# NVlabs/WarpConvNet

Measured on AMD Instinct MI355X. Metric: M active voxels/sec fwd+bwd, SparseConv3d 64→128 k=3, 1/2/4/8 MI355X, higher is better.
Workload: dtype bf16; 1 GPU; configs[1]: one 1000000-voxel uniform (U) scene per GPU, SparseConv3d 64->128 k=3, bf16 autocast, kernel-map build + AB fwd + ABt dgrad + AtB wgrad per step; voxels_per_gpu=1000000, coord_order=generator, parallelism=dp1 (scene-sharded, grad all-reduce)

## Files before the change

### warpconvnet_amd/csrc/kmap_binned.hip

```cpp
#include "kmap_cells.h"

namespace wcn {

constexpr int kInsertSample = 8;
constexpr int kInsertThreads = 512;
constexpr int kRowBufPitch = 66;
constexpr int kRowBufInts = (kCompactPitch + 1) * kRowBufPitch;
#ifndef WCN_NB_WPE
#define WCN_NB_WPE 3
#endif
constexpr int kNbWavesPerSimd = WCN_NB_WPE;
constexpr int kNbThreads = 256;

__device__ __forceinline__ int wrap_blk(int v) {
  const int bits = kBlkCoordBits;
  v &= (1 << bits) - 1;
  return (v ^ (1 << (bits - 1))) - (1 << (bits - 1));
}

__global__ void cell_prepare_kernel(uint4* __restrict__ slots, int64_t capacity, int32_t* __restrict__ ctr,
                                    uint32_t* __restrict__ halo, CellGeom g, int32_t* __restrict__ status) {
  const int64_t i = (int64_t)blockIdx.x * blockDim.x + threadIdx.x;
  if (i < capacity) slots[i] = make_uint4(0u, 0u, 0xFFFFFFFFu, 0u);
  if (i < 64) ctr[i] = 0;
  if (i == 0) *status = 0;
  if (i < g.halo_cells) {
    const int h3[3] = {g.hx, g.hy, g.hz};
    int t = (int)i, dir = 0;
    int sx = 0, sy = 0, sz = 0;
    for (; dir < 27; ++dir) {
      if (dir == 13) continue;
      const int dd[3] = {dir / 9 - 1, (dir / 3) % 3 - 1, dir % 3 - 1};
      sx = dd[0] ? h3[0] : kBlk; sy = dd[1] ? h3[1] : kBlk; sz = dd[2] ? h3[2] : kBlk;
      const int cells = sx * sy * sz;
      if (t < cells) break;
      t -= cells;
    }
    const int ddx = dir / 9 - 1, ddy = (dir / 3) % 3 - 1, ddz = dir % 3 - 1;
    const int tz = t % sz, ty = (t / sz) % sy, tx = t / (sz * sy);
    const int lx = ddx < 0 ? kBlk - g.hx + tx : tx;
    const int ly = ddy < 0 ? kBlk - g.hy + ty : ty;
    const int lz = ddz < 0 ? kBlk - g.hz + tz : tz;
    const int X = lx + kBlk * ddx + g.hx, Y = ly + kBlk * ddy + g.hy, Z = lz + kBlk * ddz + g.hz;
    halo[i] = ((uint32_t)dir << 27) | ((uint32_t)((lx * kBlk + ly) * kBlk + lz) << 16) | (uint32_t)(X * g.px + Y * g.py + Z);
  }
}

__device__ __forceinline__ void store_cell(int32_t* cell, int row, bool strict) {
  if (strict) __hip_atomic_fetch_min(reinterpret_cast<uint32_t*>(cell), (uint32_t)row, __ATOMIC_RELAXED, __HIP_MEMORY_SCOPE_AGENT);
  else *cell = row;
}

__device__ __forceinline__ int cell_of(const int4& c) {
  return ((c.y & (kBlk - 1)) * kBlk + (c.z & (kBlk - 1))) * kBlk + (c.w & (kBlk - 1));
}

template <int PHASE>
__global__ __launch_bounds__(kInsertThreads) void cell_insert_kernel(BSlot* __restrict__ slots, uint32_t cmask,
                                                          const int4* __restrict__ coords, int64_t n, CellTable t,
                                                          int32_t* __restrict__ status, int kp, int mw,
                                                          int32_t* __restrict__ nbr, uint32_t* __restrict__ mask,
                                                          int strict) {
  const bool compact = kp < 0;
  kp &= 0x7FFFFFFF;
  const int64_t tid = (int64_t)blockIdx.x * blockDim.x + threadIdx.x;
  const int64_t i = PHASE == 0 ? tid * kInsertSample : tid;
  const int lane = threadIdx.x & 63;
  bool live = i < n;
  int4 c = make_int4(0, 0, 0, 0);
  if (live) {
    c = coords[i];
    if (!coord_in_range(c.x, c.y, c.z, c.w)) {
      live = false;
      if (PHASE == 1) {
        atomicOr(status, (int)WCN_FLAG_COORD_RANGE);
        for (int k = 0; k < kp; ++k) nbr[i * kp + k] = compact ? 0 : -1;
        for (int w = 0; w < mw; ++w) mask[i * mw + w] = 0u;
      }
    }
  }
  int found = -1;
  int id = -1;
  bool created = false;
  uint64_t key = 0;
  if (live) {
    key = pack_key(c.x, c.y >> kBlkShift, c.z >> kBlkShift, c.w >> kBlkShift);
    uint32_t s = hash_slot(key, cmask);
    int idv = -1;
    for (uint32_t a = 0; a <= cmask; ++a) {
      unsigned long long* kptr = reinterpret_cast<unsigned long long*>(&slots[s].key);
      const uint4 v = *reinterpret_cast<const uint4*>(slots + s);
      unsigned long long cur = ((unsigned long long)v.y << 32) | v.x;
      if (cur == key) { found = (int)s; idv = (int)v.z; break; }
      if (cur == 0ull) {
        if (PHASE == 1) cur = __hip_atomic_load(kptr, __ATOMIC_RELAXED, __HIP_MEMORY_SCOPE_AGENT);
        if (cur == 0ull) {
          cur = atomicCAS(kptr, 0ull, (unsigned long long)key);
          if (cur == 0ull) {
            created = true;
            found = (int)s;
            break;
          }
// ... 43 lines not shown
      slots[found].id = my_id | (PHASE == 1 ? kIdLateBit : 0);
    }
    unsigned long long todo = makers;
    while (todo != 0ull) {
      const int src = __ffsll((long long)todo) - 1;
      todo &= todo - 1ull;
      const int bid = __shfl(my_id, src);
      if (bid >= 0) {
        int4* gcells = reinterpret_cast<int4*>(t.cells + (int64_t)bid * kCells);
        gcells[lane] = make_int4(-1, -1, -1, -1);
        gcells[lane + 64] = make_int4(-1, -1, -1, -1);
      }
    }
  }
  if (PHASE == 0) return;
  if (live) mask[i * mw + (mw - 1)] = (id >= 0 || found < 0) ? kMaskUnwritten : kMaskDeferred;
  if (id >= 0) store_cell(t.cells + (int64_t)id * kCells + cell_of(c), (int)i, strict != 0);
}

__global__ __launch_bounds__(256) void cell_finish_kernel(const BSlot* __restrict__ slots, uint32_t cmask,
                                                          const int4* __restrict__ coords, int64_t n, CellTable t,
                                                          CellGeom g, int mw, const uint32_t* __restrict__ mask,
                                                          int strict) {
  const int64_t tid = (int64_t)blockIdx.x * blockDim.x + threadIdx.x;
  const int64_t nthreads = (int64_t)gridDim.x * blockDim.x;
  for (int64_t i = tid; i < n; i += nthreads) {
    if (mask[i * mw + (mw - 1)] != kMaskDeferred) continue;
    const int4 c = coords[i];
    const int s = block_find(slots, cmask, pack_key(c.x, c.y >> kBlkShift, c.z >> kBlkShift, c.w >> kBlkShift));
    const int id = s >= 0 ? slots[s].id : -1;
    if (id < 0) continue;
    store_cell(t.cells + (int64_t)(id & ~kIdLateBit) * kCells + cell_of(c), (int)i, strict != 0);
  }
  const int lane = threadIdx.x & 63;
  int nblocks = t.ctr[0];
  if (nblocks > t.max_blocks) nblocks = (int)t.max_blocks;
  for (int64_t seq = tid >> 6; seq < nblocks; seq += nthreads >> 6) {
    const int id = (int)seq;
    int nid = -1;
    if (lane < 27) {
      const int ddx = lane / 9 - 1, ddy = (lane / 3) % 3 - 1, ddz = lane % 3 - 1;
      const bool needed = (ddx == 0 || g.hx > 0) && (ddy == 0 || g.hy > 0) && (ddz == 0 || g.hz > 0);
      if (lane == 13) nid = id;
      else if (needed) {
        const uint64_t key = t.blk_key[id];
        const int b = (int)((key >> 54) & kBatchMask);
        const int bx = wrap_blk((int)((key >> 36) & kCoordMask));
        const int by = wrap_blk((int)((key >> 18) & kCoordMask));
        const int bz = wrap_blk((int)(key & kCoordMask));
        const int s = block_find(slots, cmask, pack_key(b, wrap_blk(bx + ddx), wrap_blk(by + ddy), wrap_blk(bz + ddz)));
        if (s >= 0) {
          nid = slots[s].id;
          if (nid >= 0) nid &= ~kIdLateBit;
        }
      }
    }
    if (lane < 32) t.nbtab[(int64_t)id * 32 + lane] = nid;
  }
}

#ifdef WCN_PROF
__device__ unsigned long long g_bprof[4096 * 12];
#define BSTAMP(i) do { const unsigned long long now_ = wall_clock64(); prof_acc[i] += now_ - prof_prev; prof_prev = now_; } while (0)
#else
#define BSTAMP(i)
#endif

template <int LPR, bool FAST, bool COMPACT>
__global__ __launch_bounds__(kNbThreads) __attribute__((amdgpu_waves_per_eu(kNbWavesPerSimd))) void cell_neighbors_kernel(CellTable t, const uint32_t* __restrict__ halo,
                                                                    CellGeom g, int K, int kp, int mw,
                                                                    int32_t* __restrict__ nbr,
                                                                    uint32_t* __restrict__ mask,
                                                                    int32_t* __restrict__ status) {
  extern __shared__ int s_mem[];
  const int lane = threadIdx.x & 63, wave = threadIdx.x >> 6;
  uint32_t* s_halo = reinterpret_cast<uint32_t*>(s_mem);
  const int rounds = (g.halo_cells + 63) >> 6;
  const bool halo_regs = COMPACT && rounds <= 8;
  const int halo_pad = halo_regs ? 0 : rounds * 64;
  const int per_wave = g.cells + 4 + kCells / 2 + 8 + (COMPACT ? kRowBufInts : 0);
  int* s_grid = s_mem + halo_pad + wave * per_wave;
  unsigned short* s_own = reinterpret_cast<unsigned short*>(s_grid + g.cells + 4);
  const int null_cell = g.cells;
  for (int h = threadIdx.x; h < halo_pad; h += blockDim.x) s_halo[h] = h < g.halo_cells ? halo[h] : 0xFFFFFFFFu;
  if (lane == 0) s_grid[null_cell] = -1;
  __syncthreads();

  int nblocks = t.ctr[0];
  if (nblocks > t.max_blocks) nblocks = (int)t.max_blocks;
  const int gwave = blockIdx.x * (blockDim.x / 64) + wave;
  const int nwaves = gridDim.x * (blockDim.x / 64);
  constexpr int kVoxPerIter = 64 / LPR;
  const int sub = lane % LPR, vsel = lane / LPR;
  const int num_chunks = (kp + LPR - 1) / LPR;
  uint32_t he[8];
#pragma unroll
  for (int u = 0; u < 8; ++u) {
    const int idx = u * 64 + lane;
    uint32_t e = COMPACT && idx < g.halo_cells ? halo[idx] : 0xFFFFFFFFu;
    if (e == 0xFFFFFFFFu) e = (31u << 27) | (uint32_t)(g.cells + 1);
    he[u] = e;
  }
  auto load_head = [&](int seq, int& nb, int4& v0, int4& v1) {
    nb = -1;
    v0 = make_int4(-1, -1, -1, -1);
    v1 = v0;
    if (seq < nblocks) {
      if (lane < 27) nb = t.nbtab[(int64_t)seq * 32 + lane];
      const int4* own = reinterpret_cast<const int4*>(t.cells + (int64_t)seq * kCells) + lane * 2;
      v0 = own[0];
      v1 = own[1];
    }
  };
  int seq = gwave;
  int nb_c, nb_n;
  int4 c0, c1, n0, n1;
  load_head(seq, nb_c, c0, c1);
  load_head(seq + nwaves, nb_n, n0, n1);
  int hv[8];
  auto gather = [&](int nb, int r0) {
#pragma unroll
    for (int u = 0; u < 8; ++u) {
      hv[u] = -1;
      if (r0 + u < rounds) {
        const uint32_t e = s_halo[(r0 + u) * 64 + lane];
        const int nid = __shfl(nb, (int)((e >> 27) & 31u));
        if (e != 0xFFFFFFFFu && nid >= 0) hv[u] = t.cells[(int64_t)nid * kCells + ((e >> 16) & (kCells - 1))];
      }
    }
  };
  int nidv[8];
  auto gather8 = [&](int nb) {
#pragma unroll
    for (int u = 0; u < 8; ++u) nidv[u] = __shfl(nb, (int)(he[u] >> 27));
#pragma unroll
    for (int u = 0; u < 8; ++u)
      if (u < rounds) {
        const int safe = nidv[u] < 0 ? 0 : nidv[u];
        hv[u] = t.cells[(int64_t)safe * kCells + ((he[u] >> 16) & (kCells - 1))];
      }
  };
// ... 36 lines not shown
          *reinterpret_cast<int4*>(reinterpret_cast<char*>(nbr) + (__umul24((uint32_t)rid[q], kCompactPitch * 4u) + (uint32_t)piece * 16u)) = v[q];
        else
          *reinterpret_cast<int4*>(nbr + (int64_t)rid[q] * kCompactPitch + piece * 4) = v[q];
      }
    __builtin_amdgcn_fence(__ATOMIC_ACQUIRE, "wavefront");
    __builtin_amdgcn_wave_barrier();
  };
#ifdef WCN_PROF
  if (lane == 0 && gwave < 4096) g_bprof[gwave * 12 + 9] = wall_clock64();
#endif
  if (seq < nblocks) {
    if (halo_regs) gather8(nb_c);
    else gather(nb_c, 0);
  }
#ifdef WCN_PROF
  unsigned long long prof_prev = wall_clock64(), prof_acc[8] = {0, 0, 0, 0, 0, 0, 0, 0}, prof_blocks = 0;
  const unsigned long long prof_loop0 = prof_prev;
#endif
  for (; seq < nblocks; seq += nwaves) {
    BSTAMP(0);
#ifdef WCN_PROF
    ++prof_blocks;
#endif
    if (halo_regs) scatter8();
    else scatter_halo(0);
    for (int r0 = 8; r0 < rounds; r0 += 8) {
      gather(nb_c, r0);
      scatter_halo(r0);
    }
    BSTAMP(1);
    const int vals[8] = {c0.x, c0.y, c0.z, c0.w, c1.x, c1.y, c1.z, c1.w};
    const int cell0 = ((lane >> 3) + g.hx) * g.px + ((lane & 7) + g.hy) * g.py + g.hz;
    int mine = 0;
#pragma unroll
    for (int z = 0; z < 8; ++z) {
      s_grid[cell0 + z] = vals[z];
      mine += vals[z] >= 0;
    }
    int incl = mine;
#pragma unroll
    for (int d = 1; d < 64; d <<= 1) {
      const int up = __shfl_up(incl, d);
      if (lane >= d) incl += up;
    }
    const int own_cnt = __shfl(incl, 63);
    int at = incl - mine;
#pragma unroll
    for (int z = 0; z < 8; ++z)
      if (vals[z] >= 0) s_own[at++] = (unsigned short)((cell0 + z) * 4);
    if (lane < 2 * kVoxPerIter) s_own[own_cnt + lane] = (unsigned short)(null_cell * 4);
    BSTAMP(4);
    if (COMPACT) {
      flush_rows(pend_row);
      pend_row = -1;
    }
    BSTAMP(5);
    nb_c = nb_n; c0 = n0; c1 = n1;
    if (seq + nwaves < nblocks) {
      if (halo_regs) gather8(nb_c);
      else gather(nb_c, 0);
    }
    BSTAMP(6);
    load_head(seq + 2 * nwaves, nb_n, n0, n1);
    __builtin_amdgcn_fence(__ATOMIC_RELEASE, "wavefront");
    __builtin_amdgcn_wave_barrier();
    BSTAMP(2);
    const char* grid_bytes = reinterpret_cast<const char*>(s_grid);
    if (COMPACT) {
      int delta_lane = 0;
      if (lane < K) {
        const int l = lane % g.kz, j = (lane / g.kz) % g.ky, i = lane / (g.kz * g.ky);
        delta_lane = ((i - g.cx) * g.dx * g.px + (j - g.cy) * g.dy * g.py + (l - g.cz) * g.dz) * 4;
      }
      bool over = false;
      char* rows_bytes = reinterpret_cast<char*>(s_rows);
      const int origin4 = (g.hx * g.px + g.hy * g.py + g.hz) * 4;
      const uint32_t wp0 = (uint32_t)(kRowBufPitch + lane) * 4u, wp_max = (uint32_t)(kCompactPitch * kRowBufPitch + lane) * 4u;
      for (int e0 = 0; e0 < own_cnt; e0 += 64) {
        const bool live = e0 + lane < own_cnt;
        const int cell = live ? (int)s_own[e0 + lane] : origin4;
        const int row = live ? *reinterpret_cast<const int*>(grid_bytes + cell) : -1;
        uint32_t wp = wp0, rev = 0;
        auto answer = [&](int f) {
          *reinterpret_cast<int*>(rows_bytes + wp) = f;
          const uint32_t h = f >= 0 ? 1u : 0u;
          rev = (rev << 1) | h;
// ... 67 lines not shown
              if (row_a >= 0) mask[(int64_t)row_a * mw + w0 + 1] = hi_a;
              if (row_b >= 0) mask[(int64_t)row_b * mw + w0 + 1] = hi_b;
            }
          }
        }
      }
    }
    BSTAMP(3);

    __builtin_amdgcn_fence(__ATOMIC_ACQUIRE, "wavefront");
    __builtin_amdgcn_wave_barrier();
  }
  if (COMPACT) flush_rows(pend_row);
#ifdef WCN_PROF
  if (lane == 0 && gwave < 4096) {
    for (int i = 0; i < 8; ++i) g_bprof[gwave * 12 + i] = prof_acc[i];
    g_bprof[gwave * 12 + 8] = prof_blocks;
    g_bprof[gwave * 12 + 10] = prof_loop0;
    g_bprof[gwave * 12 + 11] = wall_clock64();
  }
#endif
}

static void launch_cell_table(const CellTable& t, const CellGeom& g, const int4* coords, int64_t n, int kp, int mw, int32_t* nbr,
                              uint32_t* mask, int32_t* status, int strict, hipStream_t s) {
  const int64_t capacity = t.capacity;
  const uint32_t cmask = (uint32_t)(capacity - 1);
  const int64_t max_blocks = t.max_blocks;
  const int64_t prep = capacity > g.halo_cells ? capacity : g.halo_cells;
  hipLaunchKernelGGL(cell_prepare_kernel, dim3((unsigned)ceil_div(prep, 256)), dim3(256), 0, s, (uint4*)t.slots, capacity,
                     t.ctr, t.halo, g, status);
  const int64_t n_first = ceil_div(n, kInsertSample);
  hipLaunchKernelGGL(cell_insert_kernel<0>, dim3((unsigned)ceil_div(n_first, kInsertThreads)), dim3(kInsertThreads), 0, s, t.slots, cmask,
                     coords, n, t, status, kp, mw, nbr, mask, strict);
  hipLaunchKernelGGL(cell_insert_kernel<1>, dim3((unsigned)ceil_div(n, kInsertThreads)), dim3(kInsertThreads), 0, s, t.slots, cmask,
                     coords, n, t, status, kp, mw, nbr, mask, strict);
  {
    const int64_t work = n > 64 * max_blocks ? n : 64 * max_blocks;
    int64_t wgs = ceil_div(work, 256);
    if (wgs > 8192) wgs = 8192;
    hipLaunchKernelGGL(cell_finish_kernel, dim3((unsigned)wgs), dim3(256), 0, s, (const BSlot*)t.slots, cmask,
                       coords, n, t, g, mw, (const uint32_t*)mask, strict);
  }
}

static inline int lanes_per_row_b(int kp) {
  int l = 8;
  while (l < kp && l < 64) l <<= 1;
  return l;
}

}

using namespace wcn;

extern "C" {

size_t wcn_kmap_binned_workspace(int64_t n, int64_t max_blocks) {
  if (n < 0) n = 0;
// ... 114 lines not shown
```

### warpconvnet_amd/csrc/kmap_bucket.hip

```cpp
#include "kmap_cells.h"
#include "mask_sort.h"

namespace wcn {

constexpr int kTileRows = 256;
constexpr int kBkThreads = 256;
constexpr int kTallyThreads = (kRsTile / kTileRows) * 64;
constexpr int kStageCap = 3072;

static_assert(kRsTile % kTileRows == 0, "a sort tile is a whole number of bucket tiles");
static_assert(kBkThreads == kRsThreads, "the scan launch runs rs_scan_body (mask_sort.h) in its digit workgroups");

__device__ __noinline__ void repair_row(int64_t row, const int4* __restrict__ coords, const CellTable& t, uint32_t cmask,
                                        int kp, int mw, int32_t* __restrict__ nbr, uint32_t* __restrict__ mask,
                                        int32_t* __restrict__ status) {
  const int4 c = coords[row];
  const int s = block_find(t.slots, cmask, pack_key(c.x, c.y >> kBlkShift, c.z >> kBlkShift, c.w >> kBlkShift));
  int id = s >= 0 ? t.slots[s].id : -1;
  if (id >= 0) id &= ~kIdLateBit;
  int w = -1;
  if (id >= 0) {
    const int cell = ((c.y & (kBlk - 1)) * kBlk + (c.z & (kBlk - 1))) * kBlk + (c.w & (kBlk - 1));
    w = t.cells[(int64_t)id * kCells + cell];
  }
  const bool compact = kp < 0;
  kp &= 0x7FFFFFFF;
  if (w >= 0 && w != row && !(mask[(int64_t)w * mw + (mw - 1)] & kMaskUnwritten)) {
    atomicOr(status, (int)(WCN_FLAG_DUPLICATE_COORD | (w > row ? WCN_FLAG_NEED_STRICT : 0)));
    for (int k = 0; k < kp; ++k) nbr[row * kp + k] = nbr[(int64_t)w * kp + k];
    for (int q = 0; q < mw; ++q) mask[row * mw + q] = mask[(int64_t)w * mw + q];
  } else {
    for (int k = 0; k < kp; ++k) nbr[row * kp + k] = compact ? 0 : -1;
    for (int q = 0; q < mw; ++q) mask[row * mw + q] = 0u;
  }
}

template <bool HIST, bool REPAIR>
__global__ __launch_bounds__(kTallyThreads) void kmap_tally_kernel(uint32_t* __restrict__ mask, int32_t* __restrict__ nbr,
                                                                int64_t m, int K, int kp, int mw, int64_t ntile,
                                                                int32_t* __restrict__ counts, int32_t* __restrict__ ticket,
                                                                int nblk_sort, int32_t* __restrict__ dcounts,
                                                                const int4* __restrict__ coords, CellTable t,
// ... 3 lines not shown
  const int sort_bins = 1 << sort_bits;
  const int tid = threadIdx.x, lane = tid & 63, wave = tid >> 6;
  if (HIST) {
    for (int i = tid; i < sort_bins; i += kTallyThreads) s_hist[i] = 0;
    __syncthreads();
  }
  if (blockIdx.x == 0 && tid == 0) *ticket = 0;
  constexpr int kTilesPerBlock = kRsTile / kTileRows;
  for (int tt = 0; tt < 1; ++tt) {
    const int64_t tile = (int64_t)blockIdx.x * kTilesPerBlock + wave;
    if (tile >= ntile) break;
    const int64_t row0 = tile * kTileRows;
    uint32_t last[kTileRows / 64];
#pragma unroll
    for (int sb = 0; sb < kTileRows / 64; ++sb) {
      const int64_t row = row0 + sb * 64 + lane;
      last[sb] = row < m ? mask[row * mw + (mw - 1)] : 0u;
    }
    if (REPAIR) {
#pragma unroll
      for (int sb = 0; sb < kTileRows / 64; ++sb) {
        const int64_t row = row0 + sb * 64 + lane;
        if (last[sb] & kMaskUnwritten) {
          repair_row(row, coords, t, cmask, kp, mw, nbr, mask, status);
          last[sb] = mask[row * mw + (mw - 1)];
        }
      }
    }
    for (int w = 0; w < mw; ++w) {
      const int kend = (K - w * 32) < 32 ? (K - w * 32) : 32;
      int mine = 0;
#pragma unroll
      for (int sb = 0; sb < kTileRows / 64; ++sb) {
        const int64_t row = row0 + sb * 64 + lane;
        const uint32_t bits = (w == mw - 1) ? last[sb] : (row < m ? mask[row * mw + w] : 0u);
        if (HIST && w == 0 && row < m) atomicAdd(&s_hist[rs_digit(tile_key(bits, kc), sort_shift, sort_bits)], 1);
        for (int b = 0; b < kend; ++b) {
          const int c = __popcll(__ballot((bits >> b) & 1u));
          if (lane == b) mine += c;
        }
      }
      if (lane < kend) counts[(int64_t)(w * 32 + lane) * ntile + tile] = mine;
    }
  }
  if (HIST) {
    __syncthreads();
    if ((int)blockIdx.x < nblk_sort)
// ... 581 lines not shown
```

### warpconvnet_amd/csrc/kmap_cells.h

```cpp
#pragma once

#include "wcn_common.h"

namespace wcn {

constexpr int kBlkShift = 3;
constexpr int kBlk = 1 << kBlkShift;
constexpr int kCells = kBlk * kBlk * kBlk;
constexpr int kMaxHalo = 8;
constexpr int kBlkCoordBits = kCoordBits - kBlkShift;
constexpr uint32_t kMaskUnwritten = 0x80000000u;
constexpr uint32_t kMaskDeferred = 0x80000001u;

constexpr int kCompactPitch = 16;
constexpr int kCompactIds = kCompactPitch - 1;
constexpr int kCompactFlag = (int)0x80000000;

constexpr int kIdLateBit = 1 << 30;

struct __attribute__((aligned(16))) BSlot {
  uint64_t key;
  int32_t id;
  int32_t pad;
};

struct CellTable {
  BSlot* slots;
  int64_t capacity;
  int32_t* ctr;
  uint32_t* halo;
  uint64_t* blk_key;
  int32_t* nbtab;
  int32_t* cells;
  int64_t max_blocks;
  size_t bytes;
};

struct CellGeom {
  int kx, ky, kz, cx, cy, cz, dx, dy, dz;
// ... 35 lines not shown
  g.cx = (g.kx & 1) ? g.kx / 2 : 0; g.cy = (g.ky & 1) ? g.ky / 2 : 0; g.cz = (g.kz & 1) ? g.kz / 2 : 0;
  g.dx = dilation[0]; g.dy = dilation[1]; g.dz = dilation[2];
  auto halo = [](int ks, int c, int d) { const int lo = c * d, hi = (ks - 1 - c) * d; return lo > hi ? lo : hi; };
  g.hx = halo(g.kx, g.cx, g.dx); g.hy = halo(g.ky, g.cy, g.dy); g.hz = halo(g.kz, g.cz, g.dz);
  const int gx = kBlk + 2 * g.hx, gy = kBlk + 2 * g.hy, gz = kBlk + 2 * g.hz;
  g.py = gz | 1;
  g.px = gy * g.py;
  g.cells = gx * g.px;
  g.halo_cells = gx * gy * gz - kCells;
  return g;
}

__device__ __forceinline__ int block_find(const BSlot* __restrict__ slots, uint32_t cmask, uint64_t key) {
  uint32_t s = hash_slot(key, cmask);
  for (uint32_t a = 0; a <= cmask; ++a) {
    const uint64_t k = slots[s].key;
    if (k == 0ull) return -1;
    if (k == key) return (int)s;
    s = (s + 1) & cmask;
  }
  return -1;
}

}
```

### warpconvnet_amd/csrc/kmap_stride.hip

```cpp
#include "kmap_cells.h"

namespace wcn {

constexpr int kStTile = 256;

struct StrideGeom {
  int lx, ly, lz;
};

__device__ __forceinline__ int block_id_of(const BSlot* __restrict__ slots, uint32_t cmask, const int4& c) {
  const int s = block_find(slots, cmask, pack_key(c.x, c.y >> kBlkShift, c.z >> kBlkShift, c.w >> kBlkShift));
  if (s < 0) return -1;
  const int id = slots[s].id;
  return id < 0 ? -1 : (id & ~kIdLateBit);
}

__device__ __forceinline__ int coarse_min_row(const int32_t* __restrict__ cells, int id, int x, int y, int z,
                                              const StrideGeom& g) {
  const int x0 = (x >> g.lx) << g.lx, y0 = (y >> g.ly) << g.ly, z0 = (z >> g.lz) << g.lz;
  const int32_t* sub = cells + (int64_t)id * kCells;
  int mn = 0x7FFFFFFF;
  for (int dx = 0; dx < (1 << g.lx); ++dx)
    for (int dy = 0; dy < (1 << g.ly); ++dy)
      for (int dz = 0; dz < (1 << g.lz); ++dz) {
        const int v = sub[((x0 + dx) * kBlk + (y0 + dy)) * kBlk + (z0 + dz)];
        if (v >= 0 && v < mn) mn = v;
      }
  return mn;
}

__global__ __launch_bounds__(kStTile) void stride_first_kernel(const BSlot* __restrict__ slots, uint32_t cmask, CellTable t,
                                                               const int4* __restrict__ coords, int64_t n, StrideGeom g,
                                                               unsigned long long* __restrict__ flags,
                                                               int32_t* __restrict__ counts) {
  __shared__ int s_c[kStTile / 64];
  const int64_t i = (int64_t)blockIdx.x * kStTile + threadIdx.x;
  const int lane = threadIdx.x & 63, wave = threadIdx.x >> 6;
  bool first = false;
  if (i < n) {
    const int4 c = coords[i];
    const int id = block_id_of(slots, cmask, c);
    if (id >= 0) first = coarse_min_row(t.cells, id, c.y & (kBlk - 1), c.z & (kBlk - 1), c.w & (kBlk - 1), g) == (int)i;
  }
  const unsigned long long ball = __ballot(first);
  if (lane == 0) {
    if ((int64_t)blockIdx.x * kStTile + wave * 64 < n) flags[(int64_t)blockIdx.x * (kStTile / 64) + wave] = ball;
    s_c[wave] = __popcll(ball);
  }
  __syncthreads();
  if (threadIdx.x == 0) {
    int tot = 0;
    for (int w = 0; w < kStTile / 64; ++w) tot += s_c[w];
    counts[blockIdx.x] = tot;
  }
}

__global__ __launch_bounds__(256) void stride_scan_kernel(int32_t* __restrict__ counts, int64_t ntile,
                                                          const unsigned long long* __restrict__ flags, int64_t n,
                                                          const int4* __restrict__ coords, int num_batches,
                                                          int32_t* __restrict__ out_offsets) {
  __shared__ int s_w[4];
  const int tid = threadIdx.x, lane = tid & 63, wave = tid >> 6;
  int carry = 0;
  for (int64_t base = 0; base < ntile; base += 256 * 8) {
// ... 31 lines not shown
  if (tid == 0) counts[ntile] = carry;
  __syncthreads();
  __threadfence_block();
  for (int b = tid; b <= num_batches; b += 256) {
    int64_t lo = 0, hi = n;
    while (lo < hi) {
      const int64_t mid = (lo + hi) >> 1;
      if (coords[mid].x < b) lo = mid + 1; else hi = mid;
    }
    const int64_t r = b >= num_batches ? n : lo;
    int v;
    if (r >= n) {
      v = carry;
    } else {
      const int64_t tile = r / kStTile, w0 = tile * (kStTile / 64), w1 = r >> 6;
      v = counts[tile];
      for (int64_t w = w0; w < w1; ++w) v += __popcll(flags[w]);
      v += __popcll(flags[w1] & ((1ull << (r & 63)) - 1ull));
    }
    out_offsets[b] = v;
  }
}

__global__ __launch_bounds__(kStTile) void stride_emit_kernel(const BSlot* __restrict__ slots, uint32_t cmask, CellTable t,
                                                              const int4* __restrict__ coords, int64_t n, StrideGeom g,
                                                              const unsigned long long* __restrict__ flags,
                                                              const int32_t* __restrict__ counts, int4* __restrict__ out_coords,
                                                              int32_t* __restrict__ first_rows, int K, int kp,
                                                              int32_t* __restrict__ nbr, uint32_t* __restrict__ mask) {
  const int64_t i = (int64_t)blockIdx.x * kStTile + threadIdx.x;
  const int lane = threadIdx.x & 63, wave = threadIdx.x >> 6;
  if ((int64_t)blockIdx.x * kStTile + wave * 64 >= n) return;
  const unsigned long long* fw = flags + (int64_t)blockIdx.x * (kStTile / 64);
  const unsigned long long mine = fw[wave];
  if (!((mine >> lane) & 1ull)) return;
  int pos = counts[blockIdx.x] + __popcll(mine & ((1ull << lane) - 1ull));
  for (int w = 0; w < wave; ++w) pos += __popcll(fw[w]);
  const int4 c = coords[i];
  out_coords[pos] = make_int4(c.x, c.y >> g.lx, c.z >> g.ly, c.w >> g.lz);
  if (first_rows) first_rows[pos] = (int32_t)i;
  if (!nbr) return;
  const int id = block_id_of(slots, cmask, c);
  const int x0 = ((c.y & (kBlk - 1)) >> g.lx) << g.lx, y0 = ((c.z & (kBlk - 1)) >> g.ly) << g.ly,
            z0 = ((c.w & (kBlk - 1)) >> g.lz) << g.lz;
  const int32_t* sub = t.cells + (int64_t)id * kCells;
  uint32_t bits = 0u;
  int k = 0;
  for (int dx = 0; dx < (1 << g.lx); ++dx)
    for (int dy = 0; dy < (1 << g.ly); ++dy)
      for (int dz = 0; dz < (1 << g.lz); ++dz, ++k) {
        const int v = sub[((x0 + dx) * kBlk + (y0 + dy)) * kBlk + (z0 + dz)];
        nbr[(int64_t)pos * kp + k] = v;
        if (v >= 0 && k < 32) bits |= 1u << k;
      }
  for (; k < kp; ++k) nbr[(int64_t)pos * kp + k] = -1;
  mask[pos] = bits;
}

struct CpGeom {
  int kx, ky, kz, cx, cy, cz, sx, sy, sz, dx, dy, dz;
};

template <int LPR>
__global__ __launch_bounds__(256) void cells_probe_kernel(const BSlot* __restrict__ slots, uint32_t cmask, CellTable t,
                                                          const int4* __restrict__ query, int64_t m, CpGeom g, int K,
                                                          int kp, int mw, int32_t* __restrict__ nbr,
                                                          uint32_t* __restrict__ mask) {
  constexpr int kRowsPerIter = 64 / LPR;
  const int lane = threadIdx.x & 63, wave = threadIdx.x >> 6;
  const int sub = lane % LPR, rsel = lane / LPR;
  const int64_t wave_row0 = (int64_t)blockIdx.x * 256 + wave * 64;
  const int num_chunks = (kp + LPR - 1) / LPR;
  for (int kc = 0; kc < num_chunks; ++kc) {
    const int k = kc * LPR + sub;
    const bool k_real = k < K, k_store = k < kp;
    const int l = k % g.kz, j = (k / g.kz) % g.ky, i = k / (g.kz * g.ky);
    const int ox = (i - g.cx) * g.dx, oy = (j - g.cy) * g.dy, oz = (l - g.cz) * g.dz;
#pragma unroll 4
    for (int it = 0; it < 64 / kRowsPerIter; ++it) {
      const int64_t row = wave_row0 + it * kRowsPerIter + rsel;
      int found = -1;
      if (row < m && k_real) {
        const int4 q = query[row];
        const int x = ((q.y * g.sx + ox) << (32 - kCoordBits)) >> (32 - kCoordBits);
        const int y = ((q.z * g.sy + oy) << (32 - kCoordBits)) >> (32 - kCoordBits);
        const int z = ((q.w * g.sz + oz) << (32 - kCoordBits)) >> (32 - kCoordBits);
        const int id = block_id_of(slots, cmask, make_int4(q.x, x, y, z));
        if (id >= 0)
          found = t.cells[(int64_t)id * kCells + (((x & (kBlk - 1)) * kBlk + (y & (kBlk - 1))) * kBlk + (z & (kBlk - 1)))];
      }
      if (row < m && k_store) nbr[row * kp + k] = found;
      const unsigned long long ball = __ballot(found >= 0);
      if (row < m && sub == 0) {
        const unsigned long long bits = (LPR == 64) ? ball : ((ball >> (rsel * LPR)) & ((1ull << (LPR & 63)) - 1ull));
        const int w0 = (kc * LPR) >> 5;
        if (w0 < mw) mask[row * mw + w0] = (uint32_t)bits;
        if (LPR == 64 && w0 + 1 < mw) mask[row * mw + w0 + 1] = (uint32_t)(bits >> 32);
      }
    }
  }
}

static inline int log2_stride(int s) { return s == 1 ? 0 : s == 2 ? 1 : s == 4 ? 2 : s == 8 ? 3 : -1; }

}

using namespace wcn;

extern "C" {

int wcn_cells_stride_supported(const int32_t stride[3]) {
  if (!stride) return 0;
  for (int d = 0; d < 3; ++d)
    if (log2_stride(stride[d]) < 0) return 0;
  return 1;
}

int64_t wcn_cells_stride_tiles(int64_t n) { return ceil_div(n > 0 ? n : 0, kStTile); }

int wcn_cells_stride_count(const void* cells_workspace, int64_t n, int64_t max_blocks, const int32_t* coords,
                           const int32_t stride[3], uint64_t* flags, int32_t* counts, int32_t num_batches,
                           int32_t* out_offsets, wcn_stream_t stream) {
  if (n < 0 || max_blocks < 1 || num_batches < 0 || !wcn_cells_stride_supported(stride)) return WCN_ERROR_INVALID_PARAMETERS;
  if (!cells_workspace || !flags || !counts || !out_offsets || (n > 0 && !coords) || n >= (1ll << 31))
    return WCN_ERROR_INVALID_PARAMETERS;
  hipStream_t s = (hipStream_t)stream;
  const CellTable t = carve_cells(const_cast<void*>(cells_workspace), n, max_blocks);
  const StrideGeom g{log2_stride(stride[0]), log2_stride(stride[1]), log2_stride(stride[2])};
  const int64_t ntile = wcn_cells_stride_tiles(n);
  if (ntile > 0)
    hipLaunchKernelGGL(stride_first_kernel, dim3((unsigned)ntile), dim3(kStTile), 0, s, (const BSlot*)t.slots,
                       (uint32_t)(t.capacity - 1), t, (const int4*)coords, n, g, (unsigned long long*)flags, counts);
  hipLaunchKernelGGL(stride_scan_kernel, dim3(1), dim3(256), 0, s, counts, ntile, (const unsigned long long*)flags, n,
                     (const int4*)coords, (int)num_batches, out_offsets);
  return launch_status();
}

int wcn_cells_stride_emit(const void* cells_workspace, int64_t n, int64_t max_blocks, const int32_t* coords,
                          const int32_t stride[3], const uint64_t* flags, const int32_t* counts, int32_t* out_coords,
                          int32_t* first_rows, int32_t* nbr, uint32_t* mask, wcn_stream_t stream) {
  if (n < 0 || max_blocks < 1 || !wcn_cells_stride_supported(stride)) return WCN_ERROR_INVALID_PARAMETERS;
  if (n == 0) return WCN_SUCCESS;
  if (!cells_workspace || !flags || !counts || !coords || !out_coords || n >= (1ll << 31) || ((nbr == nullptr) != (mask == nullptr)))
    return WCN_ERROR_INVALID_PARAMETERS;
  const CellTable t = carve_cells(const_cast<void*>(cells_workspace), n, max_blocks);
  const StrideGeom g{log2_stride(stride[0]), log2_stride(stride[1]), log2_stride(stride[2])};
  const int K = stride[0] * stride[1] * stride[2];
  if (nbr && K > 32) return WCN_ERROR_PROBLEM_NOT_SUPPORTED;
  hipLaunchKernelGGL(stride_emit_kernel, dim3((unsigned)wcn_cells_stride_tiles(n)), dim3(kStTile), 0, (hipStream_t)stream,
                     (const BSlot*)t.slots, (uint32_t)(t.capacity - 1), t, (const int4*)coords, n, g,
                     (const unsigned long long*)flags, counts, (int4*)out_coords, first_rows, K, (int)wcn_kmap_row_pitch(K), nbr,
                     mask);
  return launch_status();
}

int wcn_kmap_probe_cells(const void* cells_workspace, int64_t n_in, int64_t max_blocks, const int32_t* query, int64_t m,
                         const int32_t ksize[3], const int32_t stride[3], const int32_t dilation[3], int32_t* nbr,
                         uint32_t* mask, wcn_stream_t stream) {
  if (n_in < 0 || m < 0 || max_blocks < 1 || !ksize || !stride || !dilation) return WCN_ERROR_INVALID_PARAMETERS;
  for (int d = 0; d < 3; ++d)
    if (ksize[d] < 1 || stride[d] < 1 || dilation[d] < 1) return WCN_ERROR_INVALID_PARAMETERS;
  const int64_t K64 = (int64_t)ksize[0] * ksize[1] * ksize[2];
  if (K64 > 4096) return WCN_ERROR_PROBLEM_NOT_SUPPORTED;
  if (m == 0) return WCN_SUCCESS;
  if (!cells_workspace || !query || !nbr || !mask) return WCN_ERROR_INVALID_PARAMETERS;
  const int K = (int)K64, kp = wcn_kmap_row_pitch(K), mw = wcn_kmap_mask_words(K);
  const CellTable t = carve_cells(const_cast<void*>(cells_workspace), n_in, max_blocks);
  CpGeom g;
  g.kx = ksize[0]; g.ky = ksize[1]; g.kz = ksize[2];
  g.cx = (g.kx & 1) ? g.kx / 2 : 0; g.cy = (g.ky & 1) ? g.ky / 2 : 0; g.cz = (g.kz & 1) ? g.kz / 2 : 0;
  g.sx = stride[0]; g.sy = stride[1]; g.sz = stride[2];
  g.dx = dilation[0]; g.dy = dilation[1]; g.dz = dilation[2];
  const dim3 grid((unsigned)ceil_div(m, 256)), block(256);
  hipStream_t s = (hipStream_t)stream;
  const BSlot* slots = (const BSlot*)t.slots;
  const uint32_t cmask = (uint32_t)(t.capacity - 1);
  int lpr = 8;
  while (lpr < kp && lpr < 64) lpr <<= 1;
  switch (lpr) {
    case 8: hipLaunchKernelGGL(cells_probe_kernel<8>, grid, block, 0, s, slots, cmask, t, (const int4*)query, m, g, K, kp, mw, nbr, mask); break;
    case 16: hipLaunchKernelGGL(cells_probe_kernel<16>, grid, block, 0, s, slots, cmask, t, (const int4*)query, m, g, K, kp, mw, nbr, mask); break;
    case 32: hipLaunchKernelGGL(cells_probe_kernel<32>, grid, block, 0, s, slots, cmask, t, (const int4*)query, m, g, K, kp, mw, nbr, mask); break;
    default: hipLaunchKernelGGL(cells_probe_kernel<64>, grid, block, 0, s, slots, cmask, t, (const int4*)query, m, g, K, kp, mw, nbr, mask); break;
  }
  return launch_status();
}

}
```

Baseline: 1088 M voxels/s.

## Add dense bounding-box block indexing mode as alternative to hashed cell table

Result: slower. 938.0 M voxels/s (-13.7%).

```diff
diff --git a/warpconvnet_amd/csrc/kmap_binned.hip b/warpconvnet_amd/csrc/kmap_binned.hip
--- a/warpconvnet_amd/csrc/kmap_binned.hip
+++ b/warpconvnet_amd/csrc/kmap_binned.hip
@@ -1,9 +1,13 @@
+#include <stdlib.h>
+
 #include "kmap_cells.h"
 
 namespace wcn {
 
 constexpr int kInsertSample = 8;
 constexpr int kInsertThreads = 512;
+constexpr int kBoundsThreads = 512;
+constexpr int kBoundsGrid = 256;
 constexpr int kRowBufPitch = 66;
 constexpr int kRowBufInts = (kCompactPitch + 1) * kRowBufPitch;
 #ifndef WCN_NB_WPE
@@ -22,7 +26,7 @@
                                     uint32_t* __restrict__ halo, CellGeom g, int32_t* __restrict__ status) {
   const int64_t i = (int64_t)blockIdx.x * blockDim.x + threadIdx.x;
   if (i < capacity) slots[i] = make_uint4(0u, 0u, 0xFFFFFFFFu, 0u);
-  if (i < 64) ctr[i] = 0;
+  if (i < 64) ctr[i] = (i >= kCtrMin && i < kCtrMin + 4) ? 0x7FFFFFFF : (i >= kCtrMax && i < kCtrMax + 4) ? (int32_t)0x80000000 : 0;
   if (i == 0) *status = 0;
   if (i < g.halo_cells) {
     const int h3[3] = {g.hx, g.hy, g.hz};
@@ -46,6 +50,52 @@
   }
 }
 
+__global__ __launch_bounds__(kBoundsThreads) void cell_bounds_kernel(const int4* __restrict__ coords, int64_t n,
+                                                                     int32_t* __restrict__ ctr) {
+  __shared__ int s_red[kBoundsThreads / 64][8];
+  int lo[4] = {0x7FFFFFFF, 0x7FFFFFFF, 0x7FFFFFFF, 0x7FFFFFFF};
+  int hi[4] = {(int)0x80000000, (int)0x80000000, (int)0x80000000, (int)0x80000000};
+  const int64_t nthreads = (int64_t)gridDim.x * blockDim.x;
+  for (int64_t i = (int64_t)blockIdx.x * blockDim.x + threadIdx.x; i < n; i += nthreads) {
+    const int4 c = coords[i];
+    if (!coord_in_range(c.x, c.y, c.z, c.w)) continue;
+    const int v[4] = {c.x, c.y >> kBlkShift, c.z >> kBlkShift, c.w >> kBlkShift};
+#pragma unroll
+    for (int q = 0; q < 4; ++q) {
+      lo[q] = min(lo[q], v[q]);
+      hi[q] = max(hi[q], v[q]);
+    }
+  }
+#pragma unroll
+  for (int d = 32; d >= 1; d >>= 1)
+#pragma unroll
+    for (int q = 0; q < 4; ++q) {
+      lo[q] = min(lo[q], __shfl_xor(lo[q], d));
+      hi[q] = max(hi[q], __shfl_xor(hi[q], d));
+    }
+  const int lane = threadIdx.x & 63, wave = threadIdx.x >> 6;
+  if (lane == 0) {
+#pragma unroll
+    for (int q = 0; q < 4; ++q) {
+      s_red[wave][q] = lo[q];
+      s_red[wave][4 + q] = hi[q];
+    }
+  }
+  __syncthreads();
+  if (threadIdx.x < 8) {
+    const int q = threadIdx.x;
+    int v = s_red[0][q];
+    for (int w = 1; w < kBoundsThreads / 64; ++w) v = q < 4 ? min(v, s_red[w][q]) : max(v, s_red[w][q]);
+    int32_t* word = ctr + (q < 4 ? kCtrMin + q : kCtrMax + q - 4);
+    const int cur = __hip_atomic_load(word, __ATOMIC_RELAXED, __HIP_MEMORY_SCOPE_AGENT);
+    if (q < 4) {
+      if (v < cur) atomicMin(word, v);
+    } else {
+      if (v > cur) atomicMax(word, v);
+    }
+  }
+}
+
 __device__ __forceinline__ void store_cell(int32_t* cell, int row, bool strict) {
   if (strict) __hip_atomic_fetch_min(reinterpret_cast<uint32_t*>(cell), (uint32_t)row, __ATOMIC_RELAXED, __HIP_MEMORY_SCOPE_AGENT);
   else *cell = row;
@@ -60,10 +110,24 @@
                                                           const int4* __restrict__ coords, int64_t n, CellTable t,
                                                           int32_t* __restrict__ status, int kp, int mw,
                                                           int32_t* __restrict__ nbr, uint32_t* __restrict__ mask,
-                                                          int strict) {
+                                                          int strict, int box_cpv) {
   const bool compact = kp < 0;
   kp &= 0x7FFFFFFF;
   const int64_t tid = (int64_t)blockIdx.x * blockDim.x + threadIdx.x;
+  const CellBox box = PHASE == 0 ? choose_box(t.ctr, n, t.max_blocks, box_cpv) : load_box(t.ctr);
+  if (PHASE == 0 && box.mode) {
+    const int64_t blocks = (int64_t)box.nb * box.nx * box.ny * box.nz;
+    if (tid == 0) {
+      t.ctr[0] = (int32_t)blocks;
+      t.ctr[kCtrMode] = 1;
+      t.ctr[kCtrOrigin + 0] = box.b0; t.ctr[kCtrOrigin + 1] = box.x0; t.ctr[kCtrOrigin + 2] = box.y0; t.ctr[kCtrOrigin + 3] = box.z0;
+      t.ctr[kCtrDims + 0] = box.nb; t.ctr[kCtrDims + 1] = box.nx; t.ctr[kCtrDims + 2] = box.ny; t.ctr[kCtrDims + 3] = box.nz;
+    }
+    int4* all = reinterpret_cast<int4*>(t.cells);
+    const int64_t pieces = blocks * (kCells / 4), nthreads = (int64_t)gridDim.x * blockDim.x;
+    for (int64_t j = tid; j < pieces; j += nthreads) all[j] = make_int4(-1, -1, -1, -1);
+    return;
+  }
   const int64_t i = PHASE == 0 ? tid * kInsertSample : tid;
   const int lane = threadIdx.x & 63;
   bool live = i < n;
@@ -78,6 +142,14 @@
         for (int w = 0; w < mw; ++w) mask[i * mw + w] = 0u;
       }
     }
+  }
+  if (PHASE == 1 && box.mode) {
+    if (live) {
+      const int bid = box_block_id(box, c.x, c.y >> kBlkShift, c.z >> kBlkShift, c.w >> kBlkShift);
+      mask[i * mw + (mw - 1)] = kMaskUnwritten;
+      if (bid >= 0) store_cell(t.cells + (int64_t)bid * kCells + cell_of(c), (int)i, strict != 0);
+    }
+    return;
   }
   int found = -1;
   int id = -1;
@@ -167,6 +239,7 @@
                                                           const int4* __restrict__ coords, int64_t n, CellTable t,
                                                           CellGeom g, int mw, const uint32_t* __restrict__ mask,
                                                           int strict) {
+  if (t.ctr[kCtrMode]) return;
   const int64_t tid = (int64_t)blockIdx.x * blockDim.x + threadIdx.x;
   const int64_t nthreads = (int64_t)gridDim.x * blockDim.x;
   for (int64_t i = tid; i < n; i += nthreads) {
@@ -211,13 +284,11 @@
 #define BSTAMP(i)
 #endif
 
-template <int LPR, bool FAST, bool COMPACT>
-__global__ __launch_bounds__(kNbThreads) __attribute__((amdgpu_waves_per_eu(kNbWavesPerSimd))) void cell_neighbors_kernel(CellTable t, const uint32_t* __restrict__ halo,
-                                                                    CellGeom g, int K, int kp, int mw,
-                                                                    int32_t* __restrict__ nbr,
-                                                                    uint32_t* __restrict__ mask,
-                                                                    int32_t* __restrict__ status) {
-  extern __shared__ int s_mem[];
+template <int LPR, bool FAST, bool COMPACT, bool BOX>
+__device__ __forceinline__ void cell_neighbors_body(int* __restrict__ s_mem, const CellBox& box, const CellTable& t,
+                                                    const uint32_t* __restrict__ halo, const CellGeom& g, int K, int kp, int mw,
+                                                    int32_t* __restrict__ nbr, uint32_t* __restrict__ mask,
+                                                    int32_t* __restrict__ status) {
   const int lane = threadIdx.x & 63, wave = threadIdx.x >> 6;
   uint32_t* s_halo = reinterpret_cast<uint32_t*>(s_mem);
   const int rounds = (g.halo_cells + 63) >> 6;
@@ -246,22 +317,33 @@
     if (e == 0xFFFFFFFFu) e = (31u << 27) | (uint32_t)(g.cells + 1);
     he[u] = e;
   }
+  auto box_neighbor = [&](int seq) {
+    int r = __builtin_amdgcn_readfirstlane(seq);
+    const int iz = r % box.nz; r /= box.nz;
+    const int iy = r % box.ny; r /= box.ny;
+    const int ix = r % box.nx;
+    const int ddx = lane / 9 - 1, ddy = (lane / 3) % 3 - 1, ddz = lane % 3 - 1;
+    const bool in = lane < 27 && (uint32_t)(ix + ddx) < (uint32_t)box.nx && (uint32_t)(iy + ddy) < (uint32_t)box.ny &&
+                    (uint32_t)(iz + ddz) < (uint32_t)box.nz;
+    return in ? seq + (ddx * box.ny + ddy) * box.nz + ddz : -1;
+  };
   auto load_head = [&](int seq, int& nb, int4& v0, int4& v1) {
     nb = -1;
     v0 = make_int4(-1, -1, -1, -1);
     v1 = v0;
     if (seq < nblocks) {
-      if (lane < 27) nb = t.nbtab[(int64_t)seq * 32 + lane];
+      if (BOX) nb = box_neighbor(seq);
+      else if (lane < 27) nb = t.nbtab[(int64_t)seq * 32 + lane];
       const int4* own = reinterpret_cast<const int4*>(t.cells + (int64_t)seq * kCells) + lane * 2;
       v0 = own[0];
       v1 = own[1];
     }
   };
   int seq = gwave;
-  int nb_c, nb_n;
-  int4 c0, c1, n0, n1;
+  int nb_c, nb_n = -1;
+  int4 c0, c1, n0 = make_int4(-1, -1, -1, -1), n1 = n0;
   load_head(seq, nb_c, c0, c1);
-  load_head(seq + nwaves, nb_n, n0, n1);
+  if (!BOX) load_head(seq + nwaves, nb_n, n0, n1);
   int hv[8];
   auto gather = [&](int nb, int r0) {
 #pragma unroll
@@ -344,6 +426,9 @@
 #ifdef WCN_PROF
     ++prof_blocks;
 #endif
+    const bool vacant = BOX && !__any((c0.x & c0.y & c0.z & c0.w & c1.x & c1.y & c1.z & c1.w) >= 0);
+    int own_cnt = 0;
+    if (!vacant) {
     if (halo_regs) scatter8();
     else scatter_halo(0);
     for (int r0 = 8; r0 < rounds; r0 += 8) {
@@ -365,7 +450,7 @@
       const int up = __shfl_up(incl, d);
       if (lane >= d) incl += up;
     }
-    const int own_cnt = __shfl(incl, 63);
+    own_cnt = __shfl(incl, 63);
     int at = incl - mine;
 #pragma unroll
     for (int z = 0; z < 8; ++z)
@@ -377,13 +462,19 @@
       pend_row = -1;
     }
     BSTAMP(5);
-    nb_c = nb_n; c0 = n0; c1 = n1;
+    }
+    if (BOX) {
+      load_head(seq + nwaves, nb_c, c0, c1);
+    } else {
+      nb_c = nb_n; c0 = n0; c1 = n1;
+    }
     if (seq + nwaves < nblocks) {
       if (halo_regs) gather8(nb_c);
       else gather(nb_c, 0);
     }
     BSTAMP(6);
-    load_head(seq + 2 * nwaves, nb_n, n0, n1);
+    if (!BOX) load_head(seq + 2 * nwaves, nb_n, n0, n1);
+    if (vacant) continue;
     __builtin_amdgcn_fence(__ATOMIC_RELEASE, "wavefront");
     __builtin_amdgcn_wave_barrier();
     BSTAMP(2);
@@ -497,6 +588,23 @@
 #endif
 }
 
+template <int LPR, bool FAST, bool COMPACT>
+__global__ __launch_bounds__(kNbThreads) __attribute__((amdgpu_waves_per_eu(COMPACT ? kNbWavesPerSimd : 1))) void cell_neighbors_kernel(CellTable t, const uint32_t* __restrict__ halo,
+                                                                    CellGeom g, int K, int kp, int mw,
+                                                                    int32_t* __restrict__ nbr,
+                                                                    uint32_t* __restrict__ mask,
+                                                                    int32_t* __restrict__ status) {
+  extern __shared__ int s_mem[];
+  const CellBox box = load_box(t.ctr);
+  if (box.mode) cell_neighbors_body<LPR, FAST, COMPACT, true>(s_mem, box, t, halo, g, K, kp, mw, nbr, mask, status);
+  else cell_neighbors_body<LPR, FAST, COMPACT, false>(s_mem, box, t, halo, g, K, kp, mw, nbr, mask, status);
+}
+
+static int box_cells_per_voxel() {
+  const char* e = getenv("WARPCONVNET_AMD_KMAP_BOX");
+  return (e && e[0] == '1' && e[1] == 0) ? kBoxCellsPerVoxel : 0;
+}
+
 static void launch_cell_table(const CellTable& t, const CellGeom& g, const int4* coords, int64_t n, int kp, int mw, int32_t* nbr,
                               uint32_t* mask, int32_t* status, int strict, hipStream_t s) {
   const int64_t capacity = t.capacity;
@@ -505,11 +613,17 @@
   const int64_t prep = capacity > g.halo_cells ? capacity : g.halo_cells;
   hipLaunchKernelGGL(cell_prepare_kernel, dim3((unsigned)ceil_div(prep, 256)), dim3(256), 0, s, (uint4*)t.slots, capacity,
                      t.ctr, t.halo, g, status);
+  const int box_cpv = box_cells_per_voxel();
+  if (box_cpv > 0) {
+    int64_t wgs = ceil_div(n, kBoundsThreads * 4);
+    if (wgs > kBoundsGrid) wgs = kBoundsGrid;
+    hipLaunchKernelGGL(cell_bounds_kernel, dim3((unsigned)wgs), dim3(kBoundsThreads), 0, s, coords, n, t.ctr);
+  }
   const int64_t n_first = ceil_div(n, kInsertSample);
   hipLaunchKernelGGL(cell_insert_kernel<0>, dim3((unsigned)ceil_div(n_first, kInsertThreads)), dim3(kInsertThreads), 0, s, t.slots, cmask,
-                     coords, n, t, status, kp, mw, nbr, mask, strict);
+                     coords, n, t, status, kp, mw, nbr, mask, strict, box_cpv);
   hipLaunchKernelGGL(cell_insert_kernel<1>, dim3((unsigned)ceil_div(n, kInsertThreads)), dim3(kInsertThreads), 0, s, t.slots, cmask,
-                     coords, n, t, status, kp, mw, nbr, mask, strict);
+                     coords, n, t, status, kp, mw, nbr, mask, strict, box_cpv);
   {
     const int64_t work = n > 64 * max_blocks ? n : 64 * max_blocks;
     int64_t wgs = ceil_div(work, 256);
diff --git a/warpconvnet_amd/csrc/kmap_bucket.hip b/warpconvnet_amd/csrc/kmap_bucket.hip
--- a/warpconvnet_amd/csrc/kmap_bucket.hip
+++ b/warpconvnet_amd/csrc/kmap_bucket.hip
@@ -11,13 +11,11 @@
 static_assert(kRsTile % kTileRows == 0, "a sort tile is a whole number of bucket tiles");
 static_assert(kBkThreads == kRsThreads, "the scan launch runs rs_scan_body (mask_sort.h) in its digit workgroups");
 
-__device__ __noinline__ void repair_row(int64_t row, const int4* __restrict__ coords, const CellTable& t, uint32_t cmask,
+__device__ __noinline__ void repair_row(int64_t row, const int4* __restrict__ coords, const CellTable& t,
                                         int kp, int mw, int32_t* __restrict__ nbr, uint32_t* __restrict__ mask,
                                         int32_t* __restrict__ status) {
   const int4 c = coords[row];
-  const int s = block_find(t.slots, cmask, pack_key(c.x, c.y >> kBlkShift, c.z >> kBlkShift, c.w >> kBlkShift));
-  int id = s >= 0 ? t.slots[s].id : -1;
-  if (id >= 0) id &= ~kIdLateBit;
+  const int id = cell_block_id(t, load_box(t.ctr), c.x, c.y >> kBlkShift, c.z >> kBlkShift, c.w >> kBlkShift);
   int w = -1;
   if (id >= 0) {
     const int cell = ((c.y & (kBlk - 1)) * kBlk + (c.z & (kBlk - 1))) * kBlk + (c.w & (kBlk - 1));
@@ -67,7 +65,7 @@
       for (int sb = 0; sb < kTileRows / 64; ++sb) {
         const int64_t row = row0 + sb * 64 + lane;
         if (last[sb] & kMaskUnwritten) {
-          repair_row(row, coords, t, cmask, kp, mw, nbr, mask, status);
+          repair_row(row, coords, t, kp, mw, nbr, mask, status);
           last[sb] = mask[row * mw + (mw - 1)];
         }
       }
diff --git a/warpconvnet_amd/csrc/kmap_cells.h b/warpconvnet_amd/csrc/kmap_cells.h
--- a/warpconvnet_amd/csrc/kmap_cells.h
+++ b/warpconvnet_amd/csrc/kmap_cells.h
@@ -15,6 +15,13 @@
 constexpr int kCompactPitch = 16;
 constexpr int kCompactIds = kCompactPitch - 1;
 constexpr int kCompactFlag = (int)0x80000000;
+
+#ifndef WCN_BOX_CELLS_PER_VOXEL
+#define WCN_BOX_CELLS_PER_VOXEL 16
+#endif
+constexpr int kBoxCellsPerVoxel = WCN_BOX_CELLS_PER_VOXEL;
+
+constexpr int kCtrMode = 8, kCtrOrigin = 9, kCtrDims = 13, kCtrMin = 24, kCtrMax = 28;
 
 constexpr int kIdLateBit = 1 << 30;
 
@@ -96,4 +103,47 @@
   return -1;
 }
 
+struct CellBox {
+  int mode;
+  int b0, x0, y0, z0;
+  int nb, nx, ny, nz;
+};
+
+__device__ __forceinline__ CellBox choose_box(const int32_t* __restrict__ ctr, int64_t n, int64_t max_blocks, int cells_per_voxel) {
+  CellBox q;
+  q.mode = 0;
+  q.b0 = ctr[kCtrMin + 0]; q.x0 = ctr[kCtrMin + 1]; q.y0 = ctr[kCtrMin + 2]; q.z0 = ctr[kCtrMin + 3];
+  const int b1 = ctr[kCtrMax + 0], x1 = ctr[kCtrMax + 1], y1 = ctr[kCtrMax + 2], z1 = ctr[kCtrMax + 3];
+  q.nb = q.nx = q.ny = q.nz = 0;
+  if (b1 < q.b0 || x1 < q.x0 || y1 < q.y0 || z1 < q.z0) return q;
+  q.nb = b1 - q.b0 + 1; q.nx = x1 - q.x0 + 1; q.ny = y1 - q.y0 + 1; q.nz = z1 - q.z0 + 1;
+  constexpr int lo = -(1 << (kBlkCoordBits - 1)), hi = (1 << (kBlkCoordBits - 1)) - 1;
+  const bool inside = q.x0 - 1 >= lo && q.y0 - 1 >= lo && q.z0 - 1 >= lo && x1 + 1 <= hi && y1 + 1 <= hi && z1 + 1 <= hi;
+  const int64_t blocks = (int64_t)q.nb * q.nx * q.ny * q.nz;
+  if (inside && blocks <= max_blocks && blocks * kCells <= (int64_t)cells_per_voxel * n) q.mode = 1;
+  return q;
 }
+
+__device__ __forceinline__ CellBox load_box(const int32_t* __restrict__ ctr) {
+  CellBox q;
+  q.mode = ctr[kCtrMode];
+  q.b0 = ctr[kCtrOrigin + 0]; q.x0 = ctr[kCtrOrigin + 1]; q.y0 = ctr[kCtrOrigin + 2]; q.z0 = ctr[kCtrOrigin + 3];
+  q.nb = ctr[kCtrDims + 0]; q.nx = ctr[kCtrDims + 1]; q.ny = ctr[kCtrDims + 2]; q.nz = ctr[kCtrDims + 3];
+  return q;
+}
+
+__device__ __forceinline__ int box_block_id(const CellBox& q, int b, int bx, int by, int bz) {
+  const uint32_t ib = (uint32_t)(b - q.b0), ix = (uint32_t)(bx - q.x0), iy = (uint32_t)(by - q.y0), iz = (uint32_t)(bz - q.z0);
+  if (ib >= (uint32_t)q.nb || ix >= (uint32_t)q.nx || iy >= (uint32_t)q.ny || iz >= (uint32_t)q.nz) return -1;
+  return (int)(((ib * (uint32_t)q.nx + ix) * (uint32_t)q.ny + iy) * (uint32_t)q.nz + iz);
+}
+
+__device__ __forceinline__ int cell_block_id(const CellTable& t, const CellBox& q, int b, int bx, int by, int bz) {
+  if (q.mode) return box_block_id(q, b, bx, by, bz);
+  const int s = block_find(t.slots, (uint32_t)(t.capacity - 1), pack_key(b, bx, by, bz));
+  if (s < 0) return -1;
+  const int id = t.slots[s].id;
+  return id < 0 ? -1 : (id & ~kIdLateBit);
+}
+
+}
diff --git a/warpconvnet_amd/csrc/kmap_stride.hip b/warpconvnet_amd/csrc/kmap_stride.hip
--- a/warpconvnet_amd/csrc/kmap_stride.hip
+++ b/warpconvnet_amd/csrc/kmap_stride.hip
@@ -8,11 +8,8 @@
   int lx, ly, lz;
 };
 
-__device__ __forceinline__ int block_id_of(const BSlot* __restrict__ slots, uint32_t cmask, const int4& c) {
-  const int s = block_find(slots, cmask, pack_key(c.x, c.y >> kBlkShift, c.z >> kBlkShift, c.w >> kBlkShift));
-  if (s < 0) return -1;
-  const int id = slots[s].id;
-  return id < 0 ? -1 : (id & ~kIdLateBit);
+__device__ __forceinline__ int block_id_of(const CellTable& t, const CellBox& box, const int4& c) {
+  return cell_block_id(t, box, c.x, c.y >> kBlkShift, c.z >> kBlkShift, c.w >> kBlkShift);
 }
 
 __device__ __forceinline__ int coarse_min_row(const int32_t* __restrict__ cells, int id, int x, int y, int z,
@@ -29,7 +26,7 @@
   return mn;
 }
 
-__global__ __launch_bounds__(kStTile) void stride_first_kernel(const BSlot* __restrict__ slots, uint32_t cmask, CellTable t,
+__global__ __launch_bounds__(kStTile) void stride_first_kernel(CellTable t,
                                                                const int4* __restrict__ coords, int64_t n, StrideGeom g,
                                                                unsigned long long* __restrict__ flags,
                                                                int32_t* __restrict__ counts) {
@@ -39,7 +36,7 @@
   bool first = false;
   if (i < n) {
     const int4 c = coords[i];
-    const int id = block_id_of(slots, cmask, c);
+    const int id = block_id_of(t, load_box(t.ctr), c);
     if (id >= 0) first = coarse_min_row(t.cells, id, c.y & (kBlk - 1), c.z & (kBlk - 1), c.w & (kBlk - 1), g) == (int)i;
   }
   const unsigned long long ball = __ballot(first);
@@ -117,7 +114,7 @@
   }
 }
 
-__global__ __launch_bounds__(kStTile) void stride_emit_kernel(const BSlot* __restrict__ slots, uint32_t cmask, CellTable t,
+__global__ __launch_bounds__(kStTile) void stride_emit_kernel(CellTable t,
                                                               const int4* __restrict__ coords, int64_t n, StrideGeom g,
                                                               const unsigned long long* __restrict__ flags,
                                                               const int32_t* __restrict__ counts, int4* __restrict__ out_coords,
@@ -135,7 +132,7 @@
   out_coords[pos] = make_int4(c.x, c.y >> g.lx, c.z >> g.ly, c.w >> g.lz);
   if (first_rows) first_rows[pos] = (int32_t)i;
   if (!nbr) return;
-  const int id = block_id_of(slots, cmask, c);
+  const int id = block_id_of(t, load_box(t.ctr), c);
   const int x0 = ((c.y & (kBlk - 1)) >> g.lx) << g.lx, y0 = ((c.z & (kBlk - 1)) >> g.ly) << g.ly,
             z0 = ((c.w & (kBlk - 1)) >> g.lz) << g.lz;
   const int32_t* sub = t.cells + (int64_t)id * kCells;
@@ -157,7 +154,7 @@
 };
 
 template <int LPR>
-__global__ __launch_bounds__(256) void cells_probe_kernel(const BSlot* __restrict__ slots, uint32_t cmask, CellTable t,
+__global__ __launch_bounds__(256) void cells_probe_kernel(CellTable t,
                                                           const int4* __restrict__ query, int64_t m, CpGeom g, int K,
                                                           int kp, int mw, int32_t* __restrict__ nbr,
                                                           uint32_t* __restrict__ mask) {
@@ -166,6 +163,7 @@
   const int sub = lane % LPR, rsel = lane / LPR;
   const int64_t wave_row0 = (int64_t)blockIdx.x * 256 + wave * 64;
   const int num_chunks = (kp + LPR - 1) / LPR;
+  const CellBox box = load_box(t.ctr);
   for (int kc = 0; kc < num_chunks; ++kc) {
     const int k = kc * LPR + sub;
     const bool k_real = k < K, k_store = k < kp;
@@ -180,7 +178,7 @@
         const int x = ((q.y * g.sx + ox) << (32 - kCoordBits)) >> (32 - kCoordBits);
         const int y = ((q.z * g.sy + oy) << (32 - kCoordBits)) >> (32 - kCoordBits);
         const int z = ((q.w * g.sz + oz) << (32 - kCoordBits)) >> (32 - kCoordBits);
-        const int id = block_id_of(slots, cmask, make_int4(q.x, x, y, z));
+        const int id = block_id_of(t, box, make_int4(q.x, x, y, z));
         if (id >= 0)
           found = t.cells[(int64_t)id * kCells + (((x & (kBlk - 1)) * kBlk + (y & (kBlk - 1))) * kBlk + (z & (kBlk - 1)))];
       }
@@ -224,8 +222,8 @@
   const StrideGeom g{log2_stride(stride[0]), log2_stride(stride[1]), log2_stride(stride[2])};
   const int64_t ntile = wcn_cells_stride_tiles(n);
   if (ntile > 0)
-    hipLaunchKernelGGL(stride_first_kernel, dim3((unsigned)ntile), dim3(kStTile), 0, s, (const BSlot*)t.slots,
-                       (uint32_t)(t.capacity - 1), t, (const int4*)coords, n, g, (unsigned long long*)flags, counts);
+    hipLaunchKernelGGL(stride_first_kernel, dim3((unsigned)ntile), dim3(kStTile), 0, s, t, (const int4*)coords, n, g,
+                       (unsigned long long*)flags, counts);
   hipLaunchKernelGGL(stride_scan_kernel, dim3(1), dim3(256), 0, s, counts, ntile, (const unsigned long long*)flags, n,
                      (const int4*)coords, (int)num_batches, out_offsets);
   return launch_status();
@@ -243,7 +241,7 @@
   const int K = stride[0] * stride[1] * stride[2];
   if (nbr && K > 32) return WCN_ERROR_PROBLEM_NOT_SUPPORTED;
   hipLaunchKernelGGL(stride_emit_kernel, dim3((unsigned)wcn_cells_stride_tiles(n)), dim3(kStTile), 0, (hipStream_t)stream,
-                     (const BSlot*)t.slots, (uint32_t)(t.capacity - 1), t, (const int4*)coords, n, g,
+                     t, (const int4*)coords, n, g,
                      (const unsigned long long*)flags, counts, (int4*)out_coords, first_rows, K, (int)wcn_kmap_row_pitch(K), nbr,
                      mask);
   return launch_status();
@@ -268,15 +266,13 @@
   g.dx = dilation[0]; g.dy = dilation[1]; g.dz = dilation[2];
   const dim3 grid((unsigned)ceil_div(m, 256)), block(256);
   hipStream_t s = (hipStream_t)stream;
-  const BSlot* slots = (const BSlot*)t.slots;
-  const uint32_t cmask = (uint32_t)(t.capacity - 1);
   int lpr = 8;
   while (lpr < kp && lpr < 64) lpr <<= 1;
   switch (lpr) {
-    case 8: hipLaunchKernelGGL(cells_probe_kernel<8>, grid, block, 0, s, slots, cmask, t, (const int4*)query, m, g, K, kp, mw, nbr, mask); break;
-    case 16: hipLaunchKernelGGL(cells_probe_kernel<16>, grid, block, 0, s, slots, cmask, t, (const int4*)query, m, g, K, kp, mw, nbr, mask); break;
-    case 32: hipLaunchKernelGGL(cells_probe_kernel<32>, grid, block, 0, s, slots, cmask, t, (const int4*)query, m, g, K, kp, mw, nbr, mask); break;
-    default: hipLaunchKernelGGL(cells_probe_kernel<64>, grid, block, 0, s, slots, cmask, t, (const int4*)query, m, g, K, kp, mw, nbr, mask); break;
+    case 8: hipLaunchKernelGGL(cells_probe_kernel<8>, grid, block, 0, s, t, (const int4*)query, m, g, K, kp, mw, nbr, mask); break;
+    case 16: hipLaunchKernelGGL(cells_probe_kernel<16>, grid, block, 0, s, t, (const int4*)query, m, g, K, kp, mw, nbr, mask); break;
+    case 32: hipLaunchKernelGGL(cells_probe_kernel<32>, grid, block, 0, s, t, (const int4*)query, m, g, K, kp, mw, nbr, mask); break;
+    default: hipLaunchKernelGGL(cells_probe_kernel<64>, grid, block, 0, s, t, (const int4*)query, m, g, K, kp, mw, nbr, mask); break;
   }
   return launch_status();
 }
```
